# logan-pearce/olpefit

Hardware: AMD Instinct MI355X
Metric: walker-steps/sec (= model evals/sec) on 64×64 2-source cutout, 1/2/4/8 GPU (higher is better)
Workload: dtype f64

## Files before the change

### olpefit_amd/csrc/olpe.hip

```cpp
#include <hip/hip_runtime.h>

#include <limits.h>
#include <math.h>
#include <stdarg.h>
#include <stdint.h>
#include <stdio.h>
#include <stdlib.h>
#include <string.h>

#include <algorithm>
#include <cmath>
#include <atomic>
#include <vector>

#include "../../include/olpe.h"
#include "../../include/olpe_test.h"
#include "olpe_device.h"
#include "olpe_internal.h"

using namespace olpe;

namespace {

__constant__ double c_widths2[16] = {0.01, 0.01, 0.3,   0.3,    0.08,  0.09,
                                     0.0025, 0.02, 0.001, 0.0008, 0.002, 0.002,
                                     0.001, 0.001, 0.008, 0.01};
__constant__ double c_widths3[19] = {0.01,  0.01,  0.3,   0.3,  0.3,   0.3,   0.08,
                                     0.09,  0.0025, 0.02, 0.02, 0.001, 0.0008, 0.002,
                                     0.002, 0.001, 0.001, 0.008, 0.01};

template <int NSRC> __device__ __forceinline__ double width_of(int r) {
  return NSRC == 2 ? c_widths2[r] : c_widths3[r];
}

struct GibbsArgs {
  const double2 *DE;
  int n;
  int bkgd_mode;
  long long W;
  double *state;
  uint32_t *tries;
  uint32_t *accepts;
  uint32_t *mt;
  int *mt_pos;
  double *gauss;
  int *has_gauss;
  long long *done_at;
  long long n_iters;
  long long count0;
  long long burn_in;
  long long stride;
  long long row0;
  long long nrows;
  double *chain;
  long long accept_min;
  double *trace;
  unsigned long long *queue;
  unsigned long long qbase;
  int units;
  unsigned *uflag;
  unsigned utag;
  unsigned *uerr;
  unsigned long long wait_ticks;
  int balance;
  int stagger;
  unsigned *hold;
};

constexpr int kTraceF = 6;
constexpr int kSampHdr = kEtabBytes + 64;


template <int NP> struct WaveSlice {
  static constexpr int U32 = 2 * NP;
  static constexpr int PS = NP + 1;
  static constexpr int NSRC = NP == 16 ? 2 : 3;
  static constexpr int OT1 = PS, OT2 = PS + 5, OC1 = PS + 10, OC2 = PS + 13;
  static constexpr int OPT = PS + 16, OPC = PS + 21;
  static constexpr int OPR = PS + 24;
  static constexpr int F64 = 2 * PS + 24;
  static constexpr int OMD = ((U32 * 4 + F64 * 8 + 15) & ~15);
  static constexpr int OCC = (OMD + (int)sizeof(ModelDesc<NSRC>) + 15) & ~15;
  static constexpr int OPE = (OCC + 2 * NSRC * 4 * 8 + 15) & ~15;
  static constexpr int BYTES = OPE + NSRC * 2 * 64 * 8;
};
constexpr int kDrawTabBytes = (kDrawTab * 8 + 15) & ~15;
constexpr int kDrawTabExactBytes = (kThr * 8 + 15) & ~15;
__host__ __device__ constexpr int drawtab_extra(int nt, bool fast = true) {
  return (nt != 0 && nt <= 64) ? (fast ? kDrawTabBytes : kDrawTabExactBytes) : 0;
}
__host__ __device__ inline int vtab_bytes(int n, int nsrc) { return (n * 2 * nsrc * 8 + 15) & ~15; }
__host__ __device__ constexpr bool single_h(int nsrc, int nt, int wpb, bool fast) {
  return nsrc == 2 && nt == 64 && wpb == 16 && fast;
}
__host__ __device__ constexpr int sampler_vtab_bytes(int n, int nsrc, int nt, int wpb = 12,
                                                     bool fast = false) {
  return single_h(nsrc, nt, wpb, fast) ? 64 * 16
       : (nsrc == 3 && nt == 64) ? 2 * 64 * 16 : ((n * 2 * nsrc * 8 + 15) & ~15);
}
template <int NP> __host__ __device__ constexpr int ring_wave_bytes(int n) {
  return WaveSlice<NP>::OPE + kDrawTabBytes + 2 * n * 16;
}
__host__ __device__ constexpr bool ring_wpb(int nt, int wpb) {
  return nt == 128 && (wpb == 12 || wpb == 8);
}
static_assert((WaveSlice<16>::U32 * 4) % 8 == 0 && (WaveSlice<19>::U32 * 4) % 8 == 0, "align");
template <int NP> constexpr int parking_bytes() { return WaveSlice<NP>::BYTES - WaveSlice<NP>::OPE; }
static_assert(parking_bytes<16>() >= 64 * 4 * 8 && sampler_vtab_bytes(64, 2, 64) >= 64 * 4 * 8 &&
              parking_bytes<19>() >= 64 * 6 * 8 && parking_bytes<16>() >= 2 * 32 * 4 * 8 &&
              parking_bytes<19>() >= 2 * 32 * 6 * 8 && sampler_vtab_bytes(128, 2, 128) >= 128 * 4 * 8 &&
              sampler_vtab_bytes(128, 3, 128) >= 128 * 6 * 8 && drawtab_extra(32) && drawtab_extra(64),
              "sweep_exact_rows tables");

__device__ __forceinline__ Trig ld_trig(const double *s) { return Trig{s[0], s[1], s[2]}; }
__device__ __forceinline__ Coef ld_coef(const double *s) { return Coef{s[0], s[1], s[2]}; }
__device__ __forceinline__ void st_trig(double *s, const Trig &t) {
  s[0] = t.cost2; s[1] = t.sint2; s[2] = t.sin2t;
}
__device__ __forceinline__ void st_shape(double *s, const Trig &t, double ix, double iy) {
  st_trig(s, t);
  s[3] = ix; s[4] = iy;
}
__device__ __forceinline__ void st_coef(double *s, const Coef &k) {
  s[0] = k.a; s[1] = k.b; s[2] = k.c;
}

typedef __attribute__((address_space(1))) unsigned gu32;
typedef __attribute__((address_space(1))) unsigned long long gu64;
__device__ __forceinline__ void st_wt(double *p, double v) {
  __hip_atomic_store((gu64 *)p, (unsigned long long)__double_as_longlong(v), __ATOMIC_RELAXED,
                     __HIP_MEMORY_SCOPE_AGENT);
}
__device__ __forceinline__ void st_wt(long long *p, long long v) {
  __hip_atomic_store((gu64 *)p, (unsigned long long)v, __ATOMIC_RELAXED, __HIP_MEMORY_SCOPE_AGENT);
}
template <class T> __device__ __forceinline__ void st_wt(T *p, T v) {
  static_assert(sizeof(T) == 4, "32-bit word");
  unsigned u;
  __builtin_memcpy(&u, &v, 4);
  __hip_atomic_store((gu32 *)p, u, __ATOMIC_RELAXED, __HIP_MEMORY_SCOPE_AGENT);
}
template <class T> __device__ __forceinline__ T ld_uniform(const T *p) {
  static_assert(sizeof(T) == 4, "32-bit word");
  const unsigned u = (unsigned)__builtin_amdgcn_readfirstlane(
      (int)__hip_atomic_load((gu32 *)p, __ATOMIC_RELAXED, __HIP_MEMORY_SCOPE_AGENT));
  T v;
  __builtin_memcpy(&v, &u, 4);
  return v;
}
__device__ __forceinline__ void unit_publish(unsigned *flag, unsigned v, int lane) {
  asm volatile("s_waitcnt vmcnt(0)" ::: "memory");
  if (lane == 0) __hip_atomic_store((gu32 *)flag, v, __ATOMIC_RELAXED, __HIP_MEMORY_SCOPE_AGENT);
}
__device__ __forceinline__ void unit_wait(unsigned *flag, unsigned want, unsigned *err,
                                          unsigned long long *stats, int lane,
                                          unsigned long long limit, unsigned *hold) {
  const unsigned long long t0 = __builtin_amdgcn_s_memrealtime();
  bool waited = false;
  for (;;) {
    const unsigned v = (unsigned)__builtin_amdgcn_readfirstlane(
        (int)__hip_atomic_load((gu32 *)flag, __ATOMIC_RELAXED, __HIP_MEMORY_SCOPE_AGENT));
    if (v == want) break;
    if (!waited && hold && lane == 0)
      __hip_atomic_store((gu32 *)hold, 1u, __ATOMIC_RELAXED, __HIP_MEMORY_SCOPE_AGENT);
    waited = true;
    if (__builtin_amdgcn_s_memrealtime() - t0 > limit) {
      __hip_atomic_store((gu32 *)err, 1u, __ATOMIC_RELAXED, __HIP_MEMORY_SCOPE_AGENT);
      break;
    }
    __builtin_amdgcn_s_sleep(4);
  }
  if (waited && lane == 0) {
    atomicAdd(stats, 1ull);
    atomicAdd(stats + 1, __builtin_amdgcn_s_memrealtime() - t0);
  }
  __builtin_amdgcn_fence(__ATOMIC_ACQUIRE, "agent");
  asm volatile("s_waitcnt vmcnt(0)" ::: "memory");
}

__device__ __forceinline__ void hold_handoff(unsigned *hold, unsigned *err, unsigned long long limit) {
  const unsigned long long t0 = __builtin_amdgcn_s_memrealtime();
  while (__builtin_amdgcn_readfirstlane((int)__hip_atomic_load((gu32 *)hold, __ATOMIC_RELAXED,
                                                               __HIP_MEMORY_SCOPE_AGENT)) == 0) {
    if (__builtin_amdgcn_s_memrealtime() - t0 > limit) {
      __hip_atomic_store((gu32 *)err, 1u, __ATOMIC_RELAXED, __HIP_MEMORY_SCOPE_AGENT);
      break;
    }
    __builtin_amdgcn_s_sleep(4);
  }
}

constexpr int kCtrlPrio = 2;
constexpr int kGlobalWavesPerEU = 3;
template <int NSRC, int NT, bool LDS_IMG, int WPB, bool FAST>
__global__ __launch_bounds__(WPB * 64, (LDS_IMG || (NT == 128 && WPB == 12)) ? 1 : kGlobalWavesPerEU)
void olpe_gibbs_kernel(GibbsArgs A) {
  using L = Layout<NSRC>;
  using WS = WaveSlice<L::NP>;
  constexpr int NP = L::NP, PS = L::PS;
  constexpr bool RING = !LDS_IMG && FAST && ring_wpb(NT, WPB);
  using Ring = LdsRing<WPB>;
  extern __shared__ __align__(16) unsigned char smem[];
  const int n = NT ? NT : A.n;
  const int npix = n * n;
  const int lane = threadIdx.x & 63;
  const int wave = __builtin_amdgcn_readfirstlane(threadIdx.x >> 6);

  double *etab = reinterpret_cast<double *>(smem);
  unsigned *s_prog = reinterpret_cast<unsigned *>(smem + kEtabBytes);
  double2 *sDE = reinterpret_cast<double2 *>(smem + kSampHdr);
  constexpr int TABX = drawtab_extra(NT, FAST);
  const int wstride = RING ? ring_wave_bytes<NP>(n)
                           : WS::BYTES + TABX + sampler_vtab_bytes(n, NSRC, NT, WPB, FAST);
  unsigned char *wb = reinterpret_cast<unsigned char *>(sDE + (LDS_IMG ? npix : 0)) +
                      (RING ? Ring::BYTES : 0) + (size_t)wave * wstride;
  uint32_t *s_tries = reinterpret_cast<uint32_t *>(wb);
  uint32_t *s_acc = s_tries + NP;
  double *st = reinterpret_cast<double *>(wb + WS::U32 * 4);
  double *vtab = reinterpret_cast<double *>(wb + (RING ? WS::OPE + kDrawTabBytes : WS::BYTES + TABX));
  double *drawtab = reinterpret_cast<double *>(wb + (TABX ? WS::BYTES : WS::OPE));
  ModelDesc<NSRC> *mdl = reinterpret_cast<ModelDesc<NSRC> *>(wb + WS::OMD);
  double *colc = reinterpret_cast<double *>(wb + WS::OCC);

  if constexpr (LDS_IMG) {
    for (int k = threadIdx.x; k < npix; k += blockDim.x) sDE[k] = A.DE[k];
  }
  if (threadIdx.x < 64) etab[threadIdx.x] = c_exp2_64[threadIdx.x];
  if (threadIdx.x == 0) s_prog[0] = 0u;
  __syncthreads();
  const double2 *DE = LDS_IMG ? sDE : A.DE;
  [[maybe_unused]] Ring ring;
  if constexpr (RING) ring.prologue(smem + kSampHdr, A.DE, wave, lane);
  unsigned my_steps = 0;
  for (int i = 0, n = (wave >> 2) * A.stagger; i < n; ++i) __builtin_amdgcn_s_sleep(8);

  auto K = []() {
    const __attribute__((address_space(4))) GibbsArgs *p =
        (const __attribute__((address_space(4))) GibbsArgs *)__builtin_amdgcn_kernarg_segment_ptr();
    asm volatile("" : "+s"(p));
    return p;
  };

  auto take = [&]() -> int {
    unsigned long long v = 0;
    if (lane == 0) v = atomicAdd(K()->queue, 1ull) - K()->qbase;
    const unsigned d = v > 0x7fffffffull ? 0x7fffffffu : (unsigned)v;
    return __builtin_amdgcn_readfirstlane((int)d);
  };

  const int niter = (int)A.n_iters;
  const int rstride = (int)A.stride;
  const int nrows = (int)A.nrows;
  int rec_it0 = -1, rec_row0 = 0;
  if (A.stride > 0) {
    const long long c1 = A.count0 + 1;
    const long long k = c1 > A.burn_in ? (c1 - A.burn_in + A.stride - 1) / A.stride : 0;
    const long long first = A.burn_in + k * A.stride - c1;
    rec_it0 = first < niter ? (int)first : -1;
    rec_row0 = (int)(k - A.row0);
  }
  auto take_batch = [&]() -> int {
    asm volatile("s_waitcnt lgkmcnt(0)\n\ts_barrier" ::: "memory");
    if (wave == 0 && lane == 0) {
      const unsigned long long v = atomicAdd(K()->queue, 1ull) - K()->qbase;
      s_prog[1] = v > 0x7fffffffull ? 0x7fffffffu : (unsigned)v;
    }
    asm volatile("s_waitcnt lgkmcnt(0)\n\ts_barrier" ::: "memory");
    return __builtin_amdgcn_readfirstlane((int)s_prog[1]);
  };
  const int total = (int)K()->W * K()->units;
  int u = RING ? 0 : A.queue ? take() : (int)blockIdx.x * WPB + wave;
  for (;;) {
    bool active = true;
    if constexpr (RING) {
      const int bt = take_batch();
      if (bt >= (total + WPB - 1) / WPB) break;
      u = bt * WPB + wave;
      active = u < total;
      if (!active) u = 0;
    } else {
      if (u >= total) break;
    }
    const int units = K()->units;
    const int Wn = (int)K()->W;
    int w = u, k = 0, it_s = 0, it_e = niter;
    if (units > 1) {
      k = u / Wn;
      w = u - k * Wn;
      const int q = niter / units, r = niter - q * units;
      it_s = q * k + (r * k) / units;
      it_e = q * (k + 1) + (r * (k + 1)) / units;
      if (k > 0 && active)
        unit_wait(K()->uflag + w, K()->utag + (unsigned)k, K()->uerr, K()->queue + 2, lane,
                  K()->wait_ticks, K()->hold);
    }
    int it_end = it_e;
    if constexpr (RING) {
      if (lane == 0) s_prog[2 + wave] = active ? (unsigned)(it_e - it_s) : 0u;
      asm volatile("s_waitcnt lgkmcnt(0)\n\ts_barrier" ::: "memory");
      unsigned mx = 0;
      for (int j = 0; j < WPB; ++j) mx = max(mx, s_prog[2 + j]);
      it_end = it_s + (int)__builtin_amdgcn_readfirstlane((int)mx);
      if (!active) it_e = it_s;
    }
    if (lane < NP) {
      s_tries[lane] = K()->tries[(size_t)w * NP + lane];
      s_acc[lane] = K()->accepts[(size_t)w * NP + lane];
    }
    if (lane < PS) st[lane] = K()->state[(size_t)w * PS + lane];
    wave_sync();
    if (lane == 0) {
      const Trig t1 = make_trig<FAST>(st[L::T1]), t2 = make_trig<FAST>(st[L::T2]);
      st_shape(st + WS::OT1, t1, inv_var(st[L::S1X]), inv_var(st[L::S1Y]));
      st_shape(st + WS::OT2, t2, inv_var(st[L::S2X]), inv_var(st[L::S2Y]));
      st_coef(st + WS::OC1, make_coef<FAST>(st[L::S1X], st[L::S1Y], t1));
      st_coef(st + WS::OC2, make_coef<FAST>(st[L::S2X], st[L::S2Y], t2));
    }
    wave_sync();

    MTWave mt;
    mt.key = K()->mt + (size_t)w * MT_N;
    mt.pos = ld_uniform(K()->mt_pos + w);
    mt.bstart = mt.pos;
    mt.bsize = 0;
    mt.batch = 0;
    mt.has_gauss = ld_uniform(K()->has_gauss + w);
    mt.gauss = uniform_f64(K()->gauss[w]);
    mt.tab = drawtab;
    mt.thr = FAST;

    int ndone = 0;
    long long done_at = K()->done_at[w];
    if (A.accept_min > 0) {
      for (int k = 0; k < NP; ++k) ndone += (s_tries[k] >= (uint32_t)A.accept_min);
      ndone = __builtin_amdgcn_readfirstlane(ndone);
      if (ndone == NP && done_at < 0 && it_s < it_e) done_at = A.count0 + it_s + 1;
    }

    int rec_it = rec_it0, rec_row = rec_row0;
    if (rec_it0 >= 0 && it_s > rec_it0) {
      const int j = (it_s - rec_it0 + rstride - 1) / rstride;
      rec_it += j * rstride;
      rec_row += j;
    }
    double *chain_w = K()->chain + (size_t)w * nrows * PS;

    HCache hcache;
    hcache.single = single_h(NSRC, NT, WPB, FAST);
    GuardCache gcache;
    ColCache<2 * NSRC> ccache;
    ccache.pbuf = reinterpret_cast<double *>(wb + WS::OPE);
    ccache.colc = colc;
    __builtin_amdgcn_s_setprio(kCtrlPrio);
    for (int it = it_s; it < it_end; ++it) {
      if constexpr (RING) {
        if (it >= it_e) {
          ring.idle_step();
          continue;
        }
      }
      int r0 = 0, dice_idx = 0;
      double g = 0.0;
      mt.template draw<NP>(lane, 0, 2, r0, g, dice_idx);
      const int r = __builtin_amdgcn_readfirstlane(r0);
      const uint32_t tr = (uint32_t)__builtin_amdgcn_readfirstlane((int)s_tries[r]) + 1u;
      wave_sync();
      if (lane == 0) s_tries[r] = tr;
      if (A.accept_min > 0 && tr == (uint32_t)A.accept_min) {
        if (++ndone == NP && done_at < 0) done_at = A.count0 + it + 1;
      }

      const double cur = st[r];
      const double wr = width_of<NSRC>(r);
      double nv;
      if ((L::LOGMASK >> r) & 1u) {
        if constexpr (FAST) {
          const double x = (wr * g) * 2.302585092994046;
          double e;
          if (fabs(x) < 0.0625) {
            double p = fma_sc(x, 1.0 / 362880, 1.0 / 40320);
            p = fma_sc(x, p, 1.0 / 5040);
            p = fma_sc(x, p, 1.0 / 720);
            p = fma_sc(x, p, 1.0 / 120);
            p = fma_sc(x, p, 1.0 / 24);
            p = fma_sc(x, p, 1.0 / 6);
            p = fma(x, p, 0.5);
            p = fma(x, p, 1.0);
            e = fma(x, p, 1.0);
          } else {
            e = ExpTab{etab}(x);
          }
          nv = cur < 0.0 ? __builtin_nan("") : cur * e;
        } else {
          const double lv = log10(cur);
          nv = exp10(lv + wr * g);
        }
      } else {
        nv = cur + wr * g;
      }
      nv = uniform_f64(nv);

      auto q = [&](int k) -> double { return (k == r) ? nv : st[k]; };
      const int grp = (r == L::S1X || r == L::S1Y || r == L::T1) ? 1
                    : (r == L::S2X || r == L::S2Y || r == L::T2) ? 2 : 0;
      auto set_coef = [&](int ot, int isx, int isy, int ith) -> Coef {
        const Trig t = (r == ith) ? make_trig<FAST>(nv) : ld_trig(st + ot);
        Coef C;
        if constexpr (FAST) {
          double ix = st[ot + 3], iy = st[ot + 4];
          if (r == isx || r == isy) {
            const double iv = inv_var(nv);
            ix = r == isx ? iv : ix;
            iy = r == isy ? iv : iy;
          }
          C = coef_inv(t, ix, iy);
          if (lane == 0) st_shape(st + WS::OPT, t, ix, iy);
        } else {
          C = make_coef<FAST>(q(isx), q(isy), t);
          if (lane == 0) st_trig(st + WS::OPT, t);
        }
        if (lane == 0) st_coef(st + WS::OPC, C);
        return C;
      };
      Coef C1p, C2p;
      if (grp == 1) C1p = set_coef(WS::OT1, L::S1X, L::S1Y, L::T1);
      else C1p = ld_coef(st + WS::OC1);
      if (grp == 2) C2p = set_coef(WS::OT2, L::S2X, L::S2Y, L::T2);
      else C2p = ld_coef(st + WS::OC2);
      if (lane < PS) st[WS::OPR + lane] = (lane == r) ? nv : st[lane];
      wave_sync();
      if (lane < 2 * NSRC) {
        const int s = lane >> 1;
        const bool narrow = lane & 1;
        auto ql = [&](int k) -> double { return st[WS::OPR + k]; };
        const double tot = ql(L::sa(s)) - ql(L::OFF);
        const double wide = tot * ql(L::RATIO);
        const double xc = ql(L::sx(s)), yc = ql(L::sy(s));
        const Coef C{narrow ? C1p.a : C2p.a, narrow ? C1p.b : C2p.b, narrow ? C1p.c : C2p.c};
        const double dx = narrow ? 0.0 : ql(L::DX), dy = narrow ? 0.0 : ql(L::DY);
        const Gauss gq{narrow ? tot - wide : wide, narrow ? xc : xc + dx,
                       narrow ? yc : yc + dy, C};
        mdl->g[lane] = gq;
        if constexpr (FAST && NT >= 64) col_coef(gq, (double)(NT / 2), colc + 3 * lane);
        if constexpr (FAST && NT == 128) colc[6 * NSRC + lane] = ExpTab{etab}(-64.0 * gq.k.b);
      } else if (lane == 2 * NSRC) {
        mdl->bg = q(A.bkgd_mode == 0 ? L::BG_QUIRK : L::BG_FIXED);
      }
      wave_sync();

      if (LDS_IMG && K()->balance) {
        const unsigned tot = (unsigned)__builtin_amdgcn_readfirstlane((int)s_prog[0]);
        const bool behind = my_steps * (unsigned)WPB < tot;
        if (lane == 0) atomicAdd(s_prog, 1u);
        ++my_steps;
        if (behind) __builtin_amdgcn_s_setprio(1);
        else __builtin_amdgcn_s_setprio(0);
      } else {
        __builtin_amdgcn_s_setprio(0);
      }
      hcache.grp = grp;
      const unsigned gmask = gauss_mask<NSRC>(r);
      gcache.same = gmask == 0 && grp == 0;
      gcache.changed = gmask | ((grp == 1 ? 0xAAAu : grp == 2 ? 0x555u : 0u) & ((1u << (2 * NSRC)) - 1u));
      const bool nan_prop = !(nv == nv);
      double part;
      if (nan_prop) {
        gcache.same = false;
        if constexpr (RING) ring.idle_step();
        part = __builtin_nan("");
      } else {
        part = sweep<NSRC, NT, false, FAST, (WPB <= 12), Ring>(*mdl, DE, vtab, nullptr, n, lane, etab,
                                                     &hcache, &ccache, gmask, &gcache,
                                                     RING ? &ring : nullptr);
      }
      __builtin_amdgcn_s_setprio(kCtrlPrio);
      const double chi = wave_sum_v(part);

      const double dchi = chi - st[PS - 1];
      const double la = -dchi / 2.;
      const double dice = drawtab[dice_idx];
      bool acc;
      uint32_t acc_bit;
      if constexpr (FAST) {
        const double thr = drawtab[kThr + (dice_idx == 128 ? 64 : dice_idx)];
        acc_bit = (uint32_t)(__builtin_amdgcn_ballot_w64(dchi < thr) >> 32) >> 31;
      } else {
        acc_bit = (uint32_t)(__builtin_amdgcn_ballot_w64(dice < exp(la)) >> 32) >> 31;
      }
      asm volatile("" : "+s"(acc_bit));
      acc = acc_bit != 0;
      if (acc && lane == 63) st[PS - 1] = chi;
      double chi_u = 0.0, la_u = 0.0;
      if (A.trace) {
        chi_u = lane63_f64(chi);
        la_u = lane63_f64(la);
      }
      hcache.after(acc);
      gcache.after(acc);
      if constexpr (FAST && NT != 0 && NT <= 64) {
        if (acc && gmask) colcache_accept<NSRC, NT>(ccache, *mdl, gmask, lane, etab);
        ccache.pend = 0;
// ... 951 lines not shown
```

### olpefit_amd/csrc/olpe_device.h

```cpp
#pragma once
#include <hip/hip_runtime.h>
#include <stdint.h>

#include <type_traits>
#include <utility>

#include "exp_table.h"

namespace olpe {

template <int NSRC> struct Layout;

template <> struct Layout<2> {
  static constexpr int NP = 16, PS = 17;
  static constexpr int DX = 4, DY = 5, RATIO = 8, OFF = 9;
  static constexpr int S1X = 10, S1Y = 11, S2X = 12, S2Y = 13, T1 = 14, T2 = 15;
  static constexpr int BG_QUIRK = 12, BG_FIXED = 9;
  static constexpr uint32_t LOGMASK = (1u << 6) | (1u << 7) | (1u << 9) | (1u << 10) |
                                      (1u << 11) | (1u << 12) | (1u << 13);
  __device__ static constexpr int sx(int s) { return s == 0 ? 0 : 2; }
  __device__ static constexpr int sy(int s) { return s == 0 ? 1 : 3; }
  __device__ static constexpr int sa(int s) { return s == 0 ? 6 : 7; }
};

// ... 747 lines not shown
#pragma unroll
      for (int s = 1; s < NSRC; ++s) mod = mod + (Gv[2 * s] + Gv[2 * s + 1]);
      mod = mod + bg;
#pragma unroll
      for (int g = 0; g < G; ++g) {
        Gv[g] = Gv[g] * R[g];
        R[g] = R[g] * K[g];
      }
      if constexpr (WRITE) {
        if (act) out[i * n + j] = mod;
      } else {
        const double t = fma(-mod, dw.y, dw.x);
        acc = act ? fma(t, t, acc) : acc;
      }
    };
    constexpr int BLK = 4;
    const int rows = (n - cw.grp + cw.S - 1) / cw.S;
    if (!WRITE && NT != 0 && rows % BLK == 0) {
      const int rstep = cw.S * n;
      const double2 *p = DW + cw.grp * n + jj;
      double2 cur[BLK], nxt[BLK];
#pragma unroll
      for (int k = 0; k < BLK; ++k) cur[k] = p[k * rstep];
      for (int b0 = 0; b0 < rows; b0 += BLK) {
        const double2 *pn = p + ((b0 + BLK < rows) ? BLK * rstep : 0);
#pragma unroll
        for (int k = 0; k < BLK; ++k) nxt[k] = pn[k * rstep];
#pragma unroll
        for (int k = 0; k < BLK; ++k) row(cw.grp + (b0 + k) * cw.S, cur[k]);
#pragma unroll
        for (int k = 0; k < BLK; ++k) cur[k] = nxt[k];
        p = pn;
      }
    } else {
#pragma unroll 4
      for (int i = cw.grp; i < n; i += cw.S)
        row(i, WRITE ? make_double2(0.0, 0.0) : DW[i * n + jj]);
    }
  }
  return acc;
}

template <int NSRC>
__device__ __forceinline__ bool fast3_ok(const ModelDesc<NSRC> &m, int n, int rows, int kc,
                                         int lane) {
  const double hi = (double)(n - 1);
  const double S2 = (double)(row_stride(n) * row_stride(n));
  const double km = (double)(kc > rows - 1 - kc ? kc : rows - 1 - kc) + 1.0;
  const Gauss &q = m.g[lane < 2 * NSRC ? lane : 0];
  const double mx = fmax(fabs(q.x0), fabs(hi - q.x0));
  const double my = fmax(fabs(q.y0), fabs(hi - q.y0));
  const double Qb = (q.k.a * (mx * mx) + fabs(q.k.b) * mx * my) + q.k.c * (my * my);
  const double cs = q.k.c * S2;
  const bool ok = (int)(cs * km * km < 600.0) & (int)(Qb < 700.0 + cs * kc * (kc + 1.0)) &
                  (int)isfinite(Qb) & (int)isfinite(q.amp) & (int)(q.k.a >= 0.0) &
                  (int)(q.k.c >= 0.0);
  return __builtin_amdgcn_ballot_w64(!ok) == 0;
}
template <int NSRC>
__device__ __forceinline__ unsigned fast3_fails(const ModelDesc<NSRC> &m, int n, int rows,
                                                int kc, int lane) {
  const double hi = (double)(n - 1);
  const double S2 = (double)(row_stride(n) * row_stride(n));
  const double km = (double)(kc > rows - 1 - kc ? kc : rows - 1 - kc) + 1.0;
  const Gauss &q = m.g[lane < 2 * NSRC ? lane : 0];
  const double mx = fmax(fabs(q.x0), fabs(hi - q.x0));
  const double my = fmax(fabs(q.y0), fabs(hi - q.y0));
  const double Qb = (q.k.a * (mx * mx) + fabs(q.k.b) * mx * my) + q.k.c * (my * my);
  const double cs = q.k.c * S2;
  const bool ok = (int)(cs * km * km < 600.0) & (int)(Qb < 700.0 + cs * kc * (kc + 1.0)) &
                  (int)isfinite(Qb) & (int)isfinite(q.amp) & (int)(q.k.a >= 0.0) &
                  (int)(q.k.c >= 0.0);
  return (unsigned)__builtin_amdgcn_ballot_w64(!ok) & ((1u << (2 * NSRC)) - 1u);
}

template <int NSRC>
__device__ __forceinline__ bool fast3_ok_cols(const ModelDesc<NSRC> &m, int n, int rows, int kc,
                                              int lane, unsigned which) {
  const ColWalk cw(n, lane);
  const double S = (double)cw.S;
  const double kcd = (double)kc;
  const double km = (double)(kc > rows - 1 - kc ? kc : rows - 1 - kc) + 1.0;
  const double yr = (double)cw.grp;
  int ok = 1;
#pragma unroll 1
  for (unsigned f = which; f; f &= f - 1u) {
    const Gauss &q = m.g[__builtin_ctz(f)];
    const double cs = q.k.c * (S * S);
    const double K = cs * (kcd * (kcd + 1.0));
    const double amin = q.k.a - (q.k.b * q.k.b) / (4.0 * q.k.c);
    const double yd = yr - q.y0;
    ok &= (int)(cs * km * km < 600.0) & (int)(q.k.a >= 0.0) & (int)(q.k.c > 0.0) &
          (int)(fabs(q.amp) < 1e20) & (int)isfinite(amin);
#pragma unroll 1
    for (int c0 = 0; c0 < n; c0 += 64) {
      const int j = c0 + cw.jl;
      const bool act = cw.lane_ok && j < n;
      const double xd = (double)j - q.x0;
      const double bx = q.k.b * xd;
      const double q0 = (q.k.a * (xd * xd) + bx * yd) + q.k.c * (yd * yd);
      const double d0 = bx * S + (q.k.c * S) * (2.0 * yd + S);
      const double xe = K - q0;
      const double xr = d0 + 2.0 * cs * kcd;
      const int okc = (int)(fabs(xr) < 170.0) & ((int)(xe > -700.0) | (int)(amin * (xd * xd) >= 100.0));
      ok &= okc | (int)!act;
    }
  }
  return __builtin_amdgcn_ballot_w64(!ok) == 0;
}

template <int NSRC>
__device__ __forceinline__ unsigned fast3_cols_pass(const ModelDesc<NSRC> &m, int n, int rows, int kc,
                                                   int lane, unsigned which) {
  const ColWalk cw(n, lane);
  const double S = (double)cw.S;
  const double kcd = (double)kc;
  const double km = (double)(kc > rows - 1 - kc ? kc : rows - 1 - kc) + 1.0;
  const double yr = (double)cw.grp;
  unsigned passed = 0;
#pragma unroll 1
  for (unsigned f = which; f; f &= f - 1u) {
    const int g = __builtin_ctz(f);
    const Gauss &q = m.g[g];
    const double cs = q.k.c * (S * S);
    const double K = cs * (kcd * (kcd + 1.0));
    const double amin = q.k.a - (q.k.b * q.k.b) / (4.0 * q.k.c);
    const double yd = yr - q.y0;
    int ok = (int)(cs * km * km < 600.0) & (int)(q.k.a >= 0.0) & (int)(q.k.c > 0.0) &
             (int)isfinite(amin);
#pragma unroll 1
    for (int c0 = 0; c0 < n; c0 += 64) {
      const int j = c0 + cw.jl;
      const bool act = cw.lane_ok && j < n;
      const double xd = (double)j - q.x0;
      const double bx = q.k.b * xd;
      const double q0 = (q.k.a * (xd * xd) + bx * yd) + q.k.c * (yd * yd);
      const double d0 = bx * S + (q.k.c * S) * (2.0 * yd + S);
      const double xe = K - q0;
      const double xr = d0 + 2.0 * cs * kcd;
      const int okc = (int)(fabs(xr) < 170.0) & ((int)(xe > -700.0) | (int)(amin * (xd * xd) >= 100.0));
      ok &= okc | (int)!act;
    }
    if (__builtin_amdgcn_ballot_w64(!ok) == 0) passed |= 1u << g;
  }
  return passed;
}
template <int NSRC>
__device__ __forceinline__ bool fast3_amp_ok(const ModelDesc<NSRC> &m, int lane, unsigned which) {
  const bool bad = lane < 2 * NSRC && ((which >> lane) & 1u) &&
                   !(fabs(m.g[lane < 2 * NSRC ? lane : 0].amp) < 1e20);
  return __builtin_amdgcn_ballot_w64(bad) == 0;
}

__host__ __device__ constexpr bool htab_split(int nt) { return nt == 64; }
template <int NSRC, bool SPLIT = false>
__device__ __forceinline__ void build_htab(const ModelDesc<NSRC> &m, double *tab,
                                           const double *from, int which, int rows, int kc,
                                           double S, int lane, ExpTab ex) {
  const double cw2 = m.g[0].k.c * (S * S);
  const double cn2 = m.g[1].k.c * (S * S);
  for (int k = lane; k < rows; k += 64) {
    const double dk = (double)(k - kc);
    const double e = dk * (dk - 1.0);
    double2 h;
    h.x = (which & 1) ? ex(-(cw2 * e)) : from[SPLIT ? k : 2 * k];
    h.y = (which & 2) ? ex(-(cn2 * e)) : from[SPLIT ? rows + k : 2 * k + 1];
    if constexpr (SPLIT) {
      tab[k] = h.x;
      tab[rows + k] = h.y;
    } else {
      reinterpret_cast<double2 *>(tab)[k] = h;
    }
  }
  wave_sync();
}

struct GuardCache {
  bool same = false;
  bool valid = false;
  bool cur = false, prop = false;
  unsigned colok = 0, changed = 0, colprop = 0, coltest = 0;
  __device__ __forceinline__ void after(bool accepted) {
    if (same || accepted) {
      cur = prop;
      valid = true;
    }
    colok = accepted ? colprop : (colok & ~changed) | (coltest & ~changed);
    coltest = 0;
  }
};

struct HCache {
  int cur = 0;
  int valid = 0;
  int grp = 0;
  int flip = 0;
  int single = 0;
  int stale = 0;
  __device__ __forceinline__ void after(bool accepted) {
    if (single) {
      if (grp && (flip ? !accepted : accepted)) stale |= grp == 1 ? 2 : 1;
      flip = 0;
      return;
    }
    if (accepted && grp) {
      if (flip) cur ^= 1;
      else valid = false;
    }
    flip = false;
  }
};

struct ColTerm {
  double E, R;
};
__device__ __forceinline__ ColTerm col_term(const Gauss &q, double xj, double yr, double S,
                                            double kcd, ExpTab ex) {
  const double xd = xj - q.x0;
  const double yd = yr - q.y0;
  const double c = q.k.c;
  const double cs = c * (S * S);
  const double bx = q.k.b * xd;
  const double q0 = (q.k.a * (xd * xd) + bx * yd) + c * (yd * yd);
  const double d0 = bx * S + (c * S) * (2.0 * yd + S);
  return ColTerm{ex.raw(-(q0 - cs * (kcd * (kcd + 1.0)))), ex.raw(-(d0 + 2.0 * cs * kcd))};
}

__device__ __forceinline__ void col_coef(const Gauss &q, double kcd, double *cc) {
  const double yd = -q.y0;
  cc[0] = q.k.b * yd;
  cc[1] = q.k.c * (yd * yd - kcd * (kcd + 1.0));
  cc[2] = q.k.c * ((2.0 * yd + 1.0) + 2.0 * kcd);
}
__device__ __forceinline__ ColTerm col_term64(const Gauss &q, const double *cc, double xj,
                                              ExpTab ex) {
  const double xd = xj - q.x0;
  return ColTerm{ex.raw(-fma(fma(q.k.a, xd, cc[0]), xd, cc[1])), ex.raw(-fma(q.k.b, xd, cc[2]))};
}
__device__ __forceinline__ ColTerm col_term64_pass1(const Gauss &q, const double *cc, double xj,
                                                    double rho0, double step, ExpTab ex) {
  const double xd = xj - q.x0;
  return ColTerm{ex.raw(-fma(fma(q.k.a, xd, cc[0]), xd, cc[1])), rho0 * step};
}

template <int NSRC> __device__ __forceinline__ unsigned gauss_mask(int r) {
  using L = Layout<NSRC>;
  unsigned msk = 0;
#pragma unroll
  for (int s = 0; s < NSRC; ++s) {
    if (r == L::sx(s) || r == L::sy(s)) msk |= 3u << (2 * s);
    if (r == L::DX || r == L::DY || r == L::S2X || r == L::S2Y || r == L::T2) msk |= 1u << (2 * s);
    if (r == L::S1X || r == L::S1Y || r == L::T1) msk |= 2u << (2 * s);
  }
  return msk;
}

template <int G> struct ColCache {
  double E[G], R[G];
  unsigned valid = 0;
  double *pbuf = nullptr;
  unsigned pend = 0;
  const double *colc = nullptr;
};

template <int NSRC> struct MovedTerms {
  double E[NSRC], R[NSRC];
  int gi[NSRC];
  int nm;
};

template <int NSRC, int NT>
__device__ __forceinline__ void moved_terms(MovedTerms<NSRC> &mt, const ModelDesc<NSRC> &m,
                                            unsigned gmask, int n, int lane, int kc,
                                            ExpTab ex, const double *colc) {
  const ColWalk cw(n, lane);
  mt.nm = __builtin_popcount(gmask);
  unsigned rest = gmask;
#pragma unroll
  for (int k = 0; k < NSRC; ++k) {
    mt.gi[k] = rest ? __builtin_ctz(rest) : -1;
    rest &= rest - 1u;
  }
  if (mt.nm >= 2) {
#pragma unroll
    for (int k = 0; k < NSRC; ++k) {
      const int g = k < mt.nm ? mt.gi[k] : mt.gi[0];
      ColTerm t;
      if constexpr (NT == 64)
        t = col_term64(m.g[g], colc + 3 * g, (double)cw.jl, ex);
      else
        t = col_term(m.g[g], (double)cw.jl, (double)cw.grp, (double)cw.S, (double)kc, ex);
      mt.E[k] = t.E;
      mt.R[k] = t.R;
    }
  }
}

template <int NSRC, int NT, bool WRITE, bool CC = false, bool WIDE = false>
__device__ __forceinline__ double sweep_fast3(const ModelDesc<NSRC> &m, const double2 *DW,
                                              const double *htab, double *out, int n_rt,
                                              int lane, int rows, int kc, ExpTab ex,
                                              ColCache<2 * NSRC> *cc = nullptr,
                                              unsigned gmask = 0,
                                              const MovedTerms<NSRC> *pre = nullptr) {
  constexpr int G = 2 * NSRC;
  const int n = NT ? NT : n_rt;
  const ColWalk cw(n, lane);
  const double S = (double)cw.S;
  const double kcd = (double)kc;
  const double yr = (double)cw.grp;
  const double bg = m.bg;
  double acc = 0.0;
  [[maybe_unused]] double rho0[G];
  for (int c0 = 0; c0 < n; c0 += 64) {
    const int j = c0 + cw.jl;
    const bool act = cw.lane_ok && j < n;
    const double xj = (double)j;
    double av[G], rho[G];
    if constexpr (CC) {
      if (pre->nm >= 2) {
        if (cc->pbuf) {
#pragma unroll
          for (int k = 0; k < NSRC; ++k) {
            if (k < pre->nm) {
              cc->pbuf[(2 * k) * 64 + lane] = pre->E[k];
              cc->pbuf[(2 * k + 1) * 64 + lane] = pre->R[k];
            }
          }
        }
      }
    }
#pragma unroll
    for (int g = 0; g < G; ++g) {
      ColTerm t;
      if constexpr (CC) {
        const bool mine = (gmask >> g) & 1u;
        if (mine) {
          double e = pre->E[0], r = pre->R[0];
#pragma unroll
          for (int k = 1; k < NSRC; ++k) {
            e = (g == pre->gi[k]) ? pre->E[k] : e;
            r = (g == pre->gi[k]) ? pre->R[k] : r;
          }
          t = ColTerm{e, r};
        } else if ((cc->valid >> g) & 1u) {
          t = ColTerm{cc->E[g], cc->R[g]};
        } else {
          if constexpr (NT == 64)
            t = col_term64(m.g[g], cc->colc + 3 * g, xj, ex);
          else
            t = col_term(m.g[g], xj, yr, S, kcd, ex);
          cc->E[g] = t.E;
          cc->R[g] = t.R;
          cc->valid |= 1u << g;
        }
      } else if constexpr (NT == 128) {
        t = c0 == 0 ? col_term64(m.g[g], cc->colc + 3 * g, xj, ex)
                    : col_term64_pass1(m.g[g], cc->colc + 3 * g, xj, rho0[g],
                                       cc->colc[3 * G + g], ex);
        rho0[g] = t.R;
      } else if constexpr (NT >= 64) {
        t = col_term64(m.g[g], cc->colc + 3 * g, xj, ex);
      } else {
        t = col_term(m.g[g], xj, yr, S, kcd, ex);
      }
      av[g] = m.g[g].amp * t.E;
      rho[g] = t.R;
      __builtin_amdgcn_sched_barrier(0);
    }
    if constexpr (CC) cc->pend = gmask;
    const int jj = act ? j : 0;
    const double2 *hr = reinterpret_cast<const double2 *>(htab);
    auto row = [&](int i, double2 h, double2 dw) {
      double sw = av[0], sn = av[1];
#pragma unroll
      for (int s = 1; s < NSRC; ++s) {
        sw = sw + av[2 * s];
        sn = sn + av[2 * s + 1];
      }
      const double mod = fma(sn, h.y, fma(sw, h.x, bg));
#pragma unroll
      for (int g = 0; g < G; ++g) av[g] = av[g] * rho[g];
      if constexpr (WRITE) {
        if (act) out[i * n + j] = mod;
      } else {
        const double t = fma(-mod, dw.y, dw.x);
        acc = act ? fma(t, t, acc) : acc;
      }
    };
    constexpr bool LEAN = NSRC == 3 && (NT == 64 || NT == 32);
    constexpr int RU = LEAN ? 2 : 4;
    constexpr bool HPF = !LEAN;
    double rp[RU][G];
#pragma unroll
    for (int g = 0; g < G; ++g) {
      rp[1][g] = rho[g];
      if constexpr (RU == 4) {
        rp[2][g] = rho[g] * rho[g];
        rp[3][g] = rp[2][g] * rho[g];
        rp[0][g] = rp[2][g] * rp[2][g];
      } else {
        rp[0][g] = rho[g] * rho[g];
      }
    }
    auto sums4 = [&](double *sw, double *sn) __attribute__((always_inline)) {
      sw[0] = av[0];
      sn[0] = av[1];
#pragma unroll
      for (int s = 1; s < NSRC; ++s) {
        sw[0] = sw[0] + av[2 * s];
        sn[0] = sn[0] + av[2 * s + 1];
      }
#pragma unroll
      for (int r = 1; r < RU; ++r) {
        sw[r] = av[2 * NSRC - 2] * rp[r][2 * NSRC - 2];
        sn[r] = av[2 * NSRC - 1] * rp[r][2 * NSRC - 1];
#pragma unroll
        for (int s = NSRC - 2; s >= 0; --s) {
          sw[r] = fma(av[2 * s], rp[r][2 * s], sw[r]);
          sn[r] = fma(av[2 * s + 1], rp[r][2 * s + 1], sn[r]);
        }
      }
#pragma unroll
      for (int g = 0; g < G; ++g) av[g] = av[g] * rp[0][g];
    };
    auto row4 = [&](const double2 *h, const double2 *dw) {
      double sw[RU], sn[RU];
      sums4(sw, sn);
#pragma unroll
      for (int r = 0; r < RU; ++r) {
        const double mod = fma(sn[r], h[r].y, fma(sw[r], h[r].x, bg));
        const double t = fma(-mod, dw[r].y, dw[r].x);
        acc = act ? fma(t, t, acc) : acc;
      }
    };
    constexpr int BLK = 4;
    if constexpr (NT == 64 && !WRITE) {
      static_assert(htab_split(NT), "table layout");
      const double2 *p = DW + jj;
      const double *hl = htab + 64 + (lane & 15);
      double hnar[4];
#pragma unroll
      for (int q = 0; q < 4; ++q) hnar[q] = hl[16 * q];
      auto wide4 = [&](int b0, double *w) __attribute__((always_inline)) {
        const double2 a = hr[b0 / 2], b = hr[b0 / 2 + 1];
        w[0] = a.x; w[1] = a.y; w[2] = b.x; w[3] = b.y;
      };
      double2 cur[BLK], nxt[BLK];
      double hw[BLK], hwn[BLK];
#pragma unroll
      for (int k = 0; k < BLK; ++k) cur[k] = p[k * 64];
      if constexpr (HPF) wide4(0, hw);
      static_for<64 / BLK>([&](auto B) __attribute__((always_inline)) {
        constexpr int b0 = decltype(B)::value * BLK;
        constexpr bool more = b0 + BLK < 64;
        if constexpr (more) {
#pragma unroll
          for (int k = 0; k < BLK; ++k) nxt[k] = p[(b0 + BLK + k) * 64];
          if constexpr (HPF) wide4(b0 + BLK, hwn);
        }
        if constexpr (!HPF) wide4(b0, hw);
        static_for<BLK / RU>([&](auto K) __attribute__((always_inline)) {
          constexpr int r0 = b0 + decltype(K)::value * RU;
          double sw[RU], sn[RU];
          sums4(sw, sn);
          static_for<RU>([&](auto R) __attribute__((always_inline)) {
            constexpr int r = decltype(R)::value, i = r0 + r;
            double mod = fma(sw[r], hw[i - b0], bg);
            fmac_bcast_f64<i % 16>(mod, hnar[i / 16], sn[r]);
            const double t = fma(-mod, cur[i - b0].y, cur[i - b0].x);
            acc = act ? fma(t, t, acc) : acc;
          });
        });
        if constexpr (more) {
#pragma unroll
          for (int k = 0; k < BLK; ++k) {
            cur[k] = nxt[k];
            if constexpr (HPF) hw[k] = hwn[k];
          }
        }
      });
    } else if (!WRITE && NT != 0 && rows % BLK == 0) {
      const int rstep = cw.S * n;
      const double2 *p = DW + cw.grp * n + jj;
      double2 cur[BLK], nxt[BLK];
      if constexpr (!HPF) {
        double2 hc[BLK];
#pragma unroll
        for (int k = 0; k < BLK; ++k) cur[k] = p[k * rstep];
        const int R = NT >= 64 ? NT : rows;
#pragma unroll 16
        for (int b0 = 0; b0 < R; b0 += BLK) {
          const bool more = b0 + BLK < R;
          const double2 *pn = p + (more ? BLK * rstep : 0);
#pragma unroll
          for (int k = 0; k < BLK; ++k) {
            hc[k] = hr[b0 + k];
            nxt[k] = pn[k * rstep];
          }
#pragma unroll
          for (int k = 0; k < BLK; k += RU) row4(hc + k, cur + k);
#pragma unroll
          for (int k = 0; k < BLK; ++k) cur[k] = nxt[k];
          p = pn;
        }
      } else {
        double2 hc[BLK], hn[BLK];
        [[maybe_unused]] __amdgpu_buffer_rsrc_t rsrc;
        [[maybe_unused]] int voff = 0;
        if constexpr (NT > 64) {
          rsrc = __builtin_amdgcn_make_buffer_rsrc(const_cast<double2 *>(DW), (short)0,
                                                   NT * NT * 16, 0x00020000);
          voff = (cw.grp * n + jj) * 16;
        }
        auto img = [&](int r) -> double2 {
          if constexpr (NT > 64) {
            const auto v = __builtin_amdgcn_raw_buffer_load_b128(rsrc, voff, r * rstep * 16, 0);
            double2 d;
            __builtin_memcpy(&d, &v, 16);
            return d;
          } else {
            return p[r * rstep];
          }
        };
#pragma unroll
        for (int k = 0; k < BLK; ++k) {
          cur[k] = img(k);
          hc[k] = hr[k];
      }
      const int R = NT >= 64 ? NT : rows;
#pragma unroll 16
      for (int b0 = 0; b0 < R; b0 += BLK) {
        const bool more = b0 + BLK < R;
        const double2 *pn = p + (more ? BLK * rstep : 0);
        const int hb = more ? b0 + BLK : b0;
#pragma unroll
        for (int k = 0; k < BLK; ++k) {
          nxt[k] = NT > 64 ? img(hb + k) : pn[k * rstep];
          hn[k] = hr[hb + k];
        }
#pragma unroll
        for (int k = 0; k < BLK; k += RU) row4(hc + k, cur + k);
#pragma unroll
        for (int k = 0; k < BLK; ++k) {
          cur[k] = nxt[k];
          hc[k] = hn[k];
        }
        p = pn;
      }
      }
    } else {
      int k = 0;
#pragma unroll 2
      for (int i = cw.grp; i < n; i += cw.S, ++k)
        row(i, hr[k], WRITE ? make_double2(0.0, 0.0) : DW[i * n + jj]);
    }
  }
  wave_sync();
  return acc;
}


template <int WAVES> struct LdsRing {
  static constexpr int ROWS = WAVES >= 8 ? 32 : 16;
  static constexpr int SLOTS = 2, AHEAD = 1;
  static constexpr int SLOT = ROWS * 64 * 16;
  static constexpr int BYTES = SLOTS * SLOT;
  static constexpr int PPP = 128 / ROWS;
  static constexpr int PHASES = 2 * PPP;
  typedef __attribute__((address_space(3))) unsigned char lds_u8;

  const double2 *base;
  unsigned lds;
  const double2 *DW;
  unsigned g;
  int wave;
  unsigned voff;

  __device__ __forceinline__ void dma_row(int ph, int sl, int rr) const {
    const int row = (ph % PPP) * ROWS + rr;
    const double2 *src = DW + row * 128 + (ph / PPP) * 64;
    unsigned dst = lds + (unsigned)(sl * SLOT + rr * 1024);
    constexpr bool kFirstLane = WAVES != 12;
    if constexpr (kFirstLane) {
      dst = (unsigned)__builtin_amdgcn_readfirstlane((int)dst);
      src = reinterpret_cast<const double2 *>(
          (((unsigned long long)(unsigned)__builtin_amdgcn_readfirstlane(
               (int)((unsigned long long)src >> 32)))
           << 32) |
          (unsigned)__builtin_amdgcn_readfirstlane((int)(unsigned long long)src));
    }
    unsigned keep;
    asm volatile(
// ... 44 lines not shown
  const double bg = m.bg;
  const double2 *hr = reinterpret_cast<const double2 *>(htab);
  double acc = 0.0;
  double rho0[G];
#pragma unroll 1
  for (int c0 = 0; c0 < 128; c0 += 64) {
    const double xj = (double)(c0 + lane);
    double av[G], rho[G];
#pragma unroll
    for (int g = 0; g < G; ++g) {
      const ColTerm t = c0 == 0 ? col_term64(m.g[g], colc + 3 * g, xj, ex)
                                : col_term64_pass1(m.g[g], colc + 3 * g, xj, rho0[g],
                                                   colc[3 * G + g], ex);
      av[g] = m.g[g].amp * t.E;
      rho[g] = t.R;
      rho0[g] = t.R;
      __builtin_amdgcn_sched_barrier(0);
    }
    double rp[RU][G];
#pragma unroll
    for (int g = 0; g < G; ++g) {
      rp[1][g] = rho[g];
      rp[2][g] = rho[g] * rho[g];
      rp[3][g] = rp[2][g] * rho[g];
      rp[0][g] = rp[2][g] * rp[2][g];
    }
    auto row4 = [&](const double2 *h, const double2 *dw) {
      double sw[RU], sn[RU];
      sw[0] = av[0];
      sn[0] = av[1];
#pragma unroll
      for (int s = 1; s < NSRC; ++s) {
        sw[0] = sw[0] + av[2 * s];
        sn[0] = sn[0] + av[2 * s + 1];
      }
#pragma unroll
      for (int r = 1; r < RU; ++r) {
        sw[r] = av[2 * NSRC - 2] * rp[r][2 * NSRC - 2];
        sn[r] = av[2 * NSRC - 1] * rp[r][2 * NSRC - 1];
#pragma unroll
        for (int s = NSRC - 2; s >= 0; --s) {
          sw[r] = fma(av[2 * s], rp[r][2 * s], sw[r]);
          sn[r] = fma(av[2 * s + 1], rp[r][2 * s + 1], sn[r]);
        }
      }
#pragma unroll
      for (int g = 0; g < G; ++g) av[g] = av[g] * rp[0][g];
#pragma unroll
      for (int r = 0; r < RU; ++r) {
        const double mod = fma(sn[r], h[r].y, fma(sw[r], h[r].x, bg));
        const double t = fma(-mod, dw[r].y, dw[r].x);
        acc = fma(t, t, acc);
      }
    };
    const double2 *sp = ring.begin_phase();
    double2 cur[BLK], nxt[BLK], hc[BLK];
#pragma unroll
    for (int k = 0; k < BLK; ++k) cur[k] = sp[k * 64 + lane];
#pragma unroll BPP
    for (int b = 0; b < NB; ++b) {
      asm volatile("" ::: "memory");
      __builtin_amdgcn_sched_barrier(0);
#pragma unroll
      for (int k = 0; k < BLK; ++k) hc[k] = hr[b * BLK + k];
      if (b + 1 < NB) {
        const int nb = b + 1;
        if (nb % BPP == 0) sp = ring.begin_phase();
        const int r0 = (nb % BPP) * BLK;
#pragma unroll
        for (int k = 0; k < BLK; ++k) nxt[k] = sp[(r0 + k) * 64 + lane];
      }
      row4(hc, cur);
      asm volatile("" : "+v"(acc));
#pragma unroll
      for (int k = 0; k < BLK; ++k) cur[k] = nxt[k];
    }
  }
  return acc;
}

template <int NSRC, int NT>
__device__ __forceinline__ void colcache_accept(ColCache<2 * NSRC> &cc, const ModelDesc<NSRC> &m,
                                                unsigned gmask, int lane, const double *etab) {
  const ColWalk cw(NT, lane);
  const int rows0 = (NT + cw.S - 1) / cw.S;
  const double kcd = (double)(rows0 / 2);
  const bool parked = cc.pbuf && cc.pend == gmask;
#pragma unroll
  for (int g = 0; g < 2 * NSRC; ++g) {
    if ((gmask >> g) & 1u) {
      if (parked) {
        const int slot = __builtin_popcount(gmask & ((1u << g) - 1u));
        cc.E[g] = cc.pbuf[(2 * slot) * 64 + lane];
        cc.R[g] = cc.pbuf[(2 * slot + 1) * 64 + lane];
      } else {
        ColTerm t;
        if constexpr (NT == 64)
          t = col_term64(m.g[g], cc.colc + 3 * g, (double)cw.jl, ExpTab{etab});
        else
          t = col_term(m.g[g], (double)cw.jl, (double)cw.grp, (double)cw.S, kcd, ExpTab{etab});
        cc.E[g] = t.E;
        cc.R[g] = t.R;
      }
      cc.valid |= 1u << g;
    }
  }
  cc.pend = 0;
}

template <int NSRC, int NT, bool WRITE, bool FAST, bool WIDE = false, class RingT = LdsRing<12>>
__device__ __forceinline__ double sweep(const ModelDesc<NSRC> &m, const double2 *img,
                                        double *vtab, double *out, int n, int lane,
                                        const double *etab, HCache *hc = nullptr,
                                        ColCache<2 * NSRC> *cc = nullptr, unsigned gmask = 0,
                                        GuardCache *gc = nullptr, RingT *ring = nullptr) {
  if constexpr (FAST) {
    const int nn = NT ? NT : n;
    const ColWalk cw(nn, lane);
    const int rows = (nn - cw.grp + cw.S - 1) / cw.S;
    const int rows0 = (nn + cw.S - 1) / cw.S;
    const int kc = rows0 / 2;
    MovedTerms<NSRC> pre;
    if constexpr (NT != 0 && NT <= 64)
      moved_terms<NSRC, NT>(pre, m, gmask, nn, lane, kc, ExpTab{etab}, cc->colc);
    bool ok3;
    if constexpr (NT == 0 || NT > 64) {
      const unsigned fails = fast3_fails<NSRC>(m, nn, rows0, kc, lane);
      ok3 = fails == 0;
      if (!ok3) {
        asm volatile("" ::: "memory");
        if (gc) {
          const unsigned keep = gc->colok & ~gc->changed;
          const unsigned need = fails & ~keep;
          const unsigned passed = need ? fast3_cols_pass<NSRC>(m, nn, rows0, kc, lane, need) : 0u;
          gc->coltest = passed;
          gc->colprop = keep | passed;
          ok3 = (fails & ~(keep | passed)) == 0 && fast3_amp_ok<NSRC>(m, lane, fails);
        } else {
          ok3 = fast3_ok_cols<NSRC>(m, nn, rows0, kc, lane, fails);
        }
      } else if (gc) {
        gc->coltest = 0;
        gc->colprop = gc->colok & ~gc->changed;
      }
    } else {
      if (gc && gc->same && gc->valid) ok3 = gc->cur;
      else ok3 = fast3_ok<NSRC>(m, nn, rows0, kc, lane);
      if (gc) gc->prop = ok3;
    }
    asm volatile("" ::: "memory");
    if (ok3) {
      const int tw = 2 * rows0;
      const double *h;
      constexpr bool HS = htab_split(NT) && !WRITE;
      if (!hc) {
        build_htab<NSRC, HS>(m, vtab, vtab, 3, rows0, kc, (double)cw.S, lane, ExpTab{etab});
        h = vtab;
      } else if (hc->single) {
        const int need = (hc->valid ? hc->stale : 3) | (hc->grp ? (hc->grp == 1 ? 2 : 1) : 0);
        if (need)
          build_htab<NSRC, HS>(m, vtab, vtab, need, rows0, kc, (double)cw.S, lane, ExpTab{etab});
        hc->valid = 1;
        hc->stale = 0;
        hc->flip = hc->grp != 0;
        h = vtab;
      } else if (hc->grp == 0) {
        if (!hc->valid) {
          build_htab<NSRC, HS>(m, vtab + hc->cur * tw, vtab, 3, rows0, kc, (double)cw.S, lane, ExpTab{etab});
          hc->valid = true;
        }
        h = vtab + hc->cur * tw;
      } else {
        double *dst = vtab + (hc->cur ^ 1) * tw;
        build_htab<NSRC, HS>(m, dst, vtab + hc->cur * tw, hc->valid ? (hc->grp == 1 ? 2 : 1) : 3,
                         rows0, kc, (double)cw.S, lane, ExpTab{etab});
        hc->flip = true;
        h = dst;
      }
      asm volatile("" ::: "memory");
      if constexpr (NT != 0 && NT <= 64) {
        if (cc)
          return sweep_fast3<NSRC, NT, WRITE, true, WIDE>(m, img, h, out, n, lane, rows, kc,
                                                          ExpTab{etab}, cc, gmask, &pre);
      }
      if constexpr (NT == 128 && !WRITE) {
        if (ring) return sweep_fast3_ring<NSRC>(m, h, lane, ExpTab{etab}, cc->colc, *ring);
      }
      return sweep_fast3<NSRC, NT, WRITE, false, WIDE>(m, img, h, out, n, lane, rows, kc,
                                                       ExpTab{etab}, cc);
    }
    const int lvl = fast_level<NSRC>(m, nn);
    asm volatile("" ::: "memory");
    double part;
    if (lvl == 2) {
      part = sweep_fast2<NSRC, NT, WRITE>(m, img, out, n, lane);
    } else if (lvl == 1 && !(NSRC == 3 && NT == 64) && !ring && !(hc && hc->single)) {
      if (hc) hc->valid = false;
      part = sweep_fast<NSRC, NT, WRITE>(m, img, vtab, out, n, lane);
    } else {
      part = sweep_exact_dw<NSRC, NT, WRITE>(m, img, out, n, lane);
    }
    if (ring) ring->idle_step();
    return part;
  } else {
    if constexpr (!WRITE && NT == 64 && NSRC == 2) {
      if (cc) return sweep_exact_rows<NSRC, 64, true>(m, img, lane, cc->pbuf, vtab);
    } else if constexpr (!WRITE && NT == 64) {
      if (cc) return sweep_exact_rows<NSRC, 64, false>(m, img, lane, nullptr, cc->pbuf);
    } else if constexpr (!WRITE && NT == 32) {
      if (cc) return sweep_exact_rows<NSRC, 32, true>(m, img, lane, cc->pbuf, cc->pbuf + 32 * 2 * NSRC);
    } else if constexpr (!WRITE && NT == 128) {
      if (cc) return sweep_exact_rows<NSRC, 128, false>(m, img, lane, nullptr, vtab);
    }
    return sweep_exact<NSRC, NT, WRITE, 2>(m, img, out, n, lane);
  }
}

}
```

Baseline: 558.3 million.

## Use three rotating per-set shape-table slots to avoid rebuilding on reject

Replaces the single split row-shape table (with stale bits rebuilt after flip/reject) by three separate 64-entry slots, with indices for the wide and narrow sets plus a spare. A proposal that changes one group writes its new table into the spare slot, and on accept the slot indices rotate. On reject the old table stays valid, so no exp recompute is needed. It uses more LDS per wave (three 64-double slots) and adds index bookkeeping. The narrow table pointer is now passed separately into sweep_fast3.

```diff
diff --git a/olpefit_amd/csrc/olpe.hip b/olpefit_amd/csrc/olpe.hip
--- a/olpefit_amd/csrc/olpe.hip
+++ b/olpefit_amd/csrc/olpe.hip
@@ -90,14 +90,25 @@
   return (nt != 0 && nt <= 64) ? (fast ? kDrawTabBytes : kDrawTabExactBytes) : 0;
 }
 __host__ __device__ inline int vtab_bytes(int n, int nsrc) { return (n * 2 * nsrc * 8 + 15) & ~15; }
-__host__ __device__ constexpr bool single_h(int nsrc, int nt, int wpb, bool fast) {
+__host__ __device__ constexpr bool no_vtab_h(int nsrc, int nt, int wpb, bool fast) {
   return nsrc == 2 && nt == 64 && wpb == 16 && fast;
 }
+constexpr int kHsetsBytes = 3 * 64 * 8;
 __host__ __device__ constexpr int sampler_vtab_bytes(int n, int nsrc, int nt, int wpb = 12,
                                                      bool fast = false) {
-  return single_h(nsrc, nt, wpb, fast) ? 64 * 16
-       : (nsrc == 3 && nt == 64) ? 2 * 64 * 16 : ((n * 2 * nsrc * 8 + 15) & ~15);
-}
+  return (no_vtab_h(nsrc, nt, wpb, fast) || (nsrc == 3 && nt == 64))
+             ? kHsetsBytes : ((n * 2 * nsrc * 8 + 15) & ~15);
+}
+static_assert(kHsetsBytes % 16 == 0 && (64 * 8) % 16 == 0 &&
+              sampler_vtab_bytes(64, 2, 64, 12, true) >= kHsetsBytes &&
+              sampler_vtab_bytes(64, 2, 64, 8, true) >= kHsetsBytes &&
+              sampler_vtab_bytes(64, 2, 64, 16, true) == kHsetsBytes &&
+              sampler_vtab_bytes(64, 3, 64, 12, true) == kHsetsBytes, "per-set shape-table regions");
+static_assert(16 * (WaveSlice<16>::BYTES + drawtab_extra(64, true) +
+                    sampler_vtab_bytes(64, 2, 64, 16, true)) + kSampHdr + 64 * 64 * 16 <= 160 * 1024 &&
+              (WaveSlice<16>::BYTES + drawtab_extra(64, true)) % 16 == 0 &&
+              (WaveSlice<19>::BYTES + drawtab_extra(64, true)) % 16 == 0,
+              "16-wave 2-source 64x64 FAST sampler: LDS");
 template <int NP> __host__ __device__ constexpr int ring_wave_bytes(int n) {
   return WaveSlice<NP>::OPE + kDrawTabBytes + 2 * n * 16;
 }
@@ -346,7 +357,8 @@
     double *chain_w = K()->chain + (size_t)w * nrows * PS;
 
     HCache hcache;
-    hcache.single = single_h(NSRC, NT, WPB, FAST);
+    hcache.no_vtab = no_vtab_h(NSRC, NT, WPB, FAST);
+    hcache.split = FAST && htab_split(NT);
     GuardCache gcache;
     ColCache<2 * NSRC> ccache;
     ccache.pbuf = reinterpret_cast<double *>(wb + WS::OPE);
diff --git a/olpefit_amd/csrc/olpe_device.h b/olpefit_amd/csrc/olpe_device.h
--- a/olpefit_amd/csrc/olpe_device.h
+++ b/olpefit_amd/csrc/olpe_device.h
@@ -923,8 +923,7 @@
   return __builtin_amdgcn_ballot_w64(bad) == 0;
 }
 
-__host__ __device__ constexpr bool htab_split(int nt) { return nt == 64; }
-template <int NSRC, bool SPLIT = false>
+template <int NSRC>
 __device__ __forceinline__ void build_htab(const ModelDesc<NSRC> &m, double *tab,
                                            const double *from, int which, int rows, int kc,
                                            double S, int lane, ExpTab ex) {
@@ -934,14 +933,24 @@
     const double dk = (double)(k - kc);
     const double e = dk * (dk - 1.0);
     double2 h;
-    h.x = (which & 1) ? ex(-(cw2 * e)) : from[SPLIT ? k : 2 * k];
-    h.y = (which & 2) ? ex(-(cn2 * e)) : from[SPLIT ? rows + k : 2 * k + 1];
-    if constexpr (SPLIT) {
-      tab[k] = h.x;
-      tab[rows + k] = h.y;
-    } else {
-      reinterpret_cast<double2 *>(tab)[k] = h;
-    }
+    h.x = (which & 1) ? ex(-(cw2 * e)) : from[2 * k];
+    h.y = (which & 2) ? ex(-(cn2 * e)) : from[2 * k + 1];
+    reinterpret_cast<double2 *>(tab)[k] = h;
+  }
+  wave_sync();
+}
+__host__ __device__ constexpr bool htab_split(int nt) { return nt == 64; }
+template <int NSRC>
+__device__ __forceinline__ void build_hsets(const ModelDesc<NSRC> &m, double *tw, double *tn,
+                                            int which, int rows, int kc, double S, int lane,
+                                            ExpTab ex) {
+  const double cw2 = m.g[0].k.c * (S * S);
+  const double cn2 = m.g[1].k.c * (S * S);
+  for (int k = lane; k < rows; k += 64) {
+    const double dk = (double)(k - kc);
+    const double e = dk * (dk - 1.0);
+    if (which & 1) tw[k] = ex(-(cw2 * e));
+    if (which & 2) tn[k] = ex(-(cn2 * e));
   }
   wave_sync();
 }
@@ -966,11 +975,23 @@
   int valid = 0;
   int grp = 0;
   int flip = 0;
-  int single = 0;
-  int stale = 0;
+  int no_vtab = 0;
+  int split = 0;
+  int rw = 0, rn = 1;
+  __device__ __forceinline__ int spare() const { return 3 - rw - rn; }
   __device__ __forceinline__ void after(bool accepted) {
-    if (single) {
-      if (grp && (flip ? !accepted : accepted)) stale |= grp == 1 ? 2 : 1;
+    if (split) {
+      if (accepted && grp) {
+        const int bit = grp == 1 ? 2 : 1;
+        if (flip) {
+          const int sp = spare();
+          if (grp == 1) rn = sp;
+          else rw = sp;
+          valid |= bit;
+        } else {
+          valid &= ~bit;
+        }
+      }
       flip = 0;
       return;
     }
@@ -1069,8 +1090,9 @@
 
 template <int NSRC, int NT, bool WRITE, bool CC = false, bool WIDE = false>
 __device__ __forceinline__ double sweep_fast3(const ModelDesc<NSRC> &m, const double2 *DW,
-                                              const double *htab, double *out, int n_rt,
-                                              int lane, int rows, int kc, ExpTab ex,
+                                              const double *htab, const double *hnarrow,
+                                              double *out, int n_rt, int lane, int rows,
+                                              int kc, ExpTab ex,
                                               ColCache<2 * NSRC> *cc = nullptr,
                                               unsigned gmask = 0,
                                               const MovedTerms<NSRC> *pre = nullptr) {
@@ -1209,7 +1231,7 @@
     if constexpr (NT == 64 && !WRITE) {
       static_assert(htab_split(NT), "table layout");
       const double2 *p = DW + jj;
-      const double *hl = htab + 64 + (lane & 15);
+      const double *hl = hnarrow + (lane & 15);
       double hnar[4];
 #pragma unroll
       for (int q = 0; q < 4; ++q) hnar[q] = hl[16 * q];
@@ -1560,27 +1582,37 @@
     if (ok3) {
       const int tw = 2 * rows0;
       const double *h;
+      [[maybe_unused]] const double *hnar = nullptr;
       constexpr bool HS = htab_split(NT) && !WRITE;
-      if (!hc) {
-        build_htab<NSRC, HS>(m, vtab, vtab, 3, rows0, kc, (double)cw.S, lane, ExpTab{etab});
-        h = vtab;
-      } else if (hc->single) {
-        const int need = (hc->valid ? hc->stale : 3) | (hc->grp ? (hc->grp == 1 ? 2 : 1) : 0);
+      if constexpr (HS) {
+        double *dw = vtab, *dn = vtab + rows0;
+        int need = 3;
+        if (hc) {
+          const int bit = hc->grp ? (hc->grp == 1 ? 2 : 1) : 0;
+          double *sp = vtab + hc->spare() * rows0;
+          dw = bit == 1 ? sp : vtab + hc->rw * rows0;
+          dn = bit == 2 ? sp : vtab + hc->rn * rows0;
+          const int cur = ~hc->valid & 3 & ~bit;
+          need = cur | bit;
+          hc->valid |= cur;
+          hc->flip = bit != 0;
+        }
         if (need)
-          build_htab<NSRC, HS>(m, vtab, vtab, need, rows0, kc, (double)cw.S, lane, ExpTab{etab});
-        hc->valid = 1;
-        hc->stale = 0;
-        hc->flip = hc->grp != 0;
+          build_hsets<NSRC>(m, dw, dn, need, rows0, kc, (double)cw.S, lane, ExpTab{etab});
+        h = dw;
+        hnar = dn;
+      } else if (!hc) {
+        build_htab<NSRC>(m, vtab, vtab, 3, rows0, kc, (double)cw.S, lane, ExpTab{etab});
         h = vtab;
       } else if (hc->grp == 0) {
         if (!hc->valid) {
-          build_htab<NSRC, HS>(m, vtab + hc->cur * tw, vtab, 3, rows0, kc, (double)cw.S, lane, ExpTab{etab});
+          build_htab<NSRC>(m, vtab + hc->cur * tw, vtab, 3, rows0, kc, (double)cw.S, lane, ExpTab{etab});
           hc->valid = true;
         }
         h = vtab + hc->cur * tw;
       } else {
         double *dst = vtab + (hc->cur ^ 1) * tw;
-        build_htab<NSRC, HS>(m, dst, vtab + hc->cur * tw, hc->valid ? (hc->grp == 1 ? 2 : 1) : 3,
+        build_htab<NSRC>(m, dst, vtab + hc->cur * tw, hc->valid ? (hc->grp == 1 ? 2 : 1) : 3,
                          rows0, kc, (double)cw.S, lane, ExpTab{etab});
         hc->flip = true;
         h = dst;
@@ -1588,13 +1620,13 @@
       asm volatile("" ::: "memory");
       if constexpr (NT != 0 && NT <= 64) {
         if (cc)
-          return sweep_fast3<NSRC, NT, WRITE, true, WIDE>(m, img, h, out, n, lane, rows, kc,
-                                                          ExpTab{etab}, cc, gmask, &pre);
+          return sweep_fast3<NSRC, NT, WRITE, true, WIDE>(m, img, h, hnar, out, n, lane, rows,
+                                                          kc, ExpTab{etab}, cc, gmask, &pre);
       }
       if constexpr (NT == 128 && !WRITE) {
         if (ring) return sweep_fast3_ring<NSRC>(m, h, lane, ExpTab{etab}, cc->colc, *ring);
       }
-      return sweep_fast3<NSRC, NT, WRITE, false, WIDE>(m, img, h, out, n, lane, rows, kc,
+      return sweep_fast3<NSRC, NT, WRITE, false, WIDE>(m, img, h, hnar, out, n, lane, rows, kc,
                                                        ExpTab{etab}, cc);
     }
     const int lvl = fast_level<NSRC>(m, nn);
@@ -1602,7 +1634,7 @@
     double part;
     if (lvl == 2) {
       part = sweep_fast2<NSRC, NT, WRITE>(m, img, out, n, lane);
-    } else if (lvl == 1 && !(NSRC == 3 && NT == 64) && !ring && !(hc && hc->single)) {
+    } else if (lvl == 1 && !(NSRC == 3 && NT == 64) && !ring && !(hc && hc->no_vtab)) {
       if (hc) hc->valid = false;
       part = sweep_fast<NSRC, NT, WRITE>(m, img, vtab, out, n, lane);
     } else {
```

After: 560.9 million (median of 6 runs). About the same (+0.5%).
